# maxgillett/tinysplat

Measured on AMD Instinct MI355X. Metric: Gaussians*pixels/s fwd+bwd, higher is better.
Workload: dtype f32; 1 GPU; 1000000 random Gaussians, SH degree 3, 1920x1080, fwd+bwd (RGB), BASELINE configs[2]; max_per_tile=614, parallelism=single GPU, tile_lists=16x16 (gsplat's) (auto), gaussian_order=as generated (i.i.d.)

## Files before the change

### tinysplat_amd/csrc/raster.hip

```cpp
#include <hip/hip_runtime.h>

#include <type_traits>

#include "../../include/tinysplat_hip.h"
#include "host_util.h"
#include "raster_survivors.h"
#include "splat_math.h"

namespace {
#include "sort_network.h"

#ifndef TS_FWD_MIN_WAVES_RGB
#define TS_FWD_MIN_WAVES_RGB 5
#endif
#ifndef TS_FWD_MIN_WAVES_RGBD
#define TS_FWD_MIN_WAVES_RGBD 5
#endif
#ifndef TS_BWD_MIN_WAVES_16
#define TS_BWD_MIN_WAVES_16 5
#endif

#ifndef TS_ABLATE
#define TS_ABLATE 0
#endif

#ifndef TS_STATS
#define TS_STATS 0
#endif
#if TS_STATS
__device__ unsigned long long ts_stats[12];
#define TS_STAT(i, v)                                                                       \
    do {                                                                                    \
        if ((threadIdx.x & 63) == 0) atomicAdd(&ts_stats[i], (unsigned long long)(v));      \
    } while (0)
#else
#define TS_STAT(i, v) ((void)0)
#endif

#ifndef TS_TIMELINE
#define TS_TIMELINE 0
#endif
#if TS_TIMELINE
constexpr int kTimelineMax = 1 << 17;
constexpr int kTimelineRow = 12;
__device__ unsigned long long ts_timeline[2][kTimelineMax][kTimelineRow];
struct WaveClock {
    unsigned long long t0, c0;
    unsigned long long seg[4] = {0ull, 0ull, 0ull, 0ull};
    unsigned int work[3] = {0u, 0u, 0u};
    int which, unit, n;
    __device__ WaveClock(int which_, int unit_, int n_) : which(which_), unit(unit_), n(n_) {
        t0 = __builtin_amdgcn_s_memrealtime();
        c0 = __builtin_amdgcn_s_memtime();
    }
    __device__ ~WaveClock() {
        const unsigned long long t1 = __builtin_amdgcn_s_memrealtime();
        const unsigned long long c1 = __builtin_amdgcn_s_memtime();
        unsigned hw, xcc;
        asm volatile("s_getreg_b32 %0, hwreg(HW_REG_HW_ID)" : "=s"(hw));
        asm volatile("s_getreg_b32 %0, hwreg(HW_REG_XCC_ID)" : "=s"(xcc));
        if ((threadIdx.x & 63) == 0 && unit < kTimelineMax) {
            ts_timeline[which][unit][0] = t0;
            ts_timeline[which][unit][1] = t1;
            ts_timeline[which][unit][2] = (unsigned long long)hw | ((unsigned long long)xcc << 32);
            ts_timeline[which][unit][3] = (unsigned long long)n;
            for (int i = 0; i < 4; ++i) ts_timeline[which][unit][4 + i] = seg[i];
            ts_timeline[which][unit][8] = c1 - c0;
            for (int i = 0; i < 3; ++i) ts_timeline[which][unit][9 + i] = work[i];
        }
    }
};
#define TS_WAVE_CLOCK(which, unit, n) WaveClock ts_wave_clock_(which, unit, n)
#define TS_SEG_PARAM , unsigned long long (&ts_seg_)[4], unsigned int (&ts_work_)[3]
#define TS_SEG_ARG , ts_wave_clock_.seg, ts_wave_clock_.work
#define TS_WORK(i, v) ts_work_[i] += (unsigned int)(v)
#define TS_SEG_T0(var)                                               \
    __builtin_amdgcn_sched_barrier(0);                               \
    const unsigned long long var = __builtin_amdgcn_s_memtime();     \
    __builtin_amdgcn_sched_barrier(0)
#define TS_SEG_ADD(segs, i, var)                                     \
    __builtin_amdgcn_sched_barrier(0);                               \
    segs[i] += __builtin_amdgcn_s_memtime() - var;                   \
    __builtin_amdgcn_sched_barrier(0)
#else
#define TS_WAVE_CLOCK(which, unit, n) ((void)0)
#define TS_SEG_PARAM
#define TS_SEG_ARG
#define TS_WORK(i, v) ((void)0)
#define TS_SEG_T0(var) ((void)0)
#define TS_SEG_ADD(segs, i, var) ((void)0)
#endif

#ifndef TS_LDS_PAD
#define TS_LDS_PAD 0
#endif
#if TS_LDS_PAD
#define TS_LDS_PAD_DECL() __shared__ int lds_pad_[TS_LDS_PAD / 4]; if (threadIdx.x == 9999) lds_pad_[blockIdx.x & 7] = 1; asm volatile("" : : "v"(&lds_pad_[0]) : "memory")
#else
#define TS_LDS_PAD_DECL() ((void)0)
#endif

typedef __attribute__((address_space(3))) void* lds_ptr_t;
typedef const __attribute__((address_space(1))) void* gbl_ptr_t;
__device__ __forceinline__ void dma_record(const float4* __restrict__ splats, int g, float4* raw) {
    const float4* p = splats + 3 * (size_t)g;
    __builtin_amdgcn_global_load_lds((gbl_ptr_t)p, (lds_ptr_t)raw, 16, 0, 0);
    __builtin_amdgcn_global_load_lds((gbl_ptr_t)(p + 1), (lds_ptr_t)(raw + 64), 16, 0, 0);
    __builtin_amdgcn_global_load_lds((gbl_ptr_t)(p + 2), (lds_ptr_t)(raw + 128), 16, 0, 0);
}
#define TS_DMA_WAIT() asm volatile("s_waitcnt vmcnt(0)" ::: "memory")
#define TS_LDS_WAIT() asm volatile("s_waitcnt lgkmcnt(0)" ::: "memory")

#ifndef TS_REDUCE_AHEAD
#define TS_REDUCE_AHEAD 4
#endif

constexpr int kWaves = 4;
constexpr int kThreads = 64 * kWaves;
constexpr int kRowF4 = TS_PARTIAL_ROW_FLOATS / 4;
static_assert(TS_PARTIAL_ROW_FLOATS % 4 == 0 && TS_PARTIAL_ROW_FLOATS >= 12, "row = whole float4s, >= 10 values");
using ts::kLog2e;
using ts::kLog2_255;

#define TS_WAVE_SYNC()                                            \
    do {                                                          \
        __builtin_amdgcn_fence(__ATOMIC_RELEASE, "wavefront");    \
        __builtin_amdgcn_wave_barrier();                          \
        __builtin_amdgcn_fence(__ATOMIC_ACQUIRE, "wavefront");    \
    } while (0)

#define TS_LDS_BARRIER() asm volatile("s_waitcnt lgkmcnt(0)\n\ts_barrier" ::: "memory")

__device__ __forceinline__ int wave_max_int(int v) {
#pragma unroll
    for (int d = 32; d >= 1; d >>= 1) v = max(v, __shfl_xor(v, d, 64));
    return v;
}

__device__ __forceinline__ float sigma_l2(float hA, float B, float hC, float neg_lo, float dx, float dy) {
    float s = __builtin_fmaf(hC * dy, dy, neg_lo);
    s = __builtin_fmaf(hA * dx, dx, s);
    return __builtin_fmaf(B * dx, dy, s);
}

__device__ __forceinline__ int xcd_tile_group(int num_groups) {
    const int per_xcd = (num_groups + 7) >> 3;
    return (int)(blockIdx.x & 7) * per_xcd + (int)(blockIdx.x >> 3);
}

struct Staged {
    int mask;
    float gx, gy, hA, B, hC, lo;
};

struct BlockRect { float x0, x1, y0, y1; };
__device__ __forceinline__ bool mask_rect(unsigned long long m, int& xmin, int& xmax, int& ymin,
                                          int& ymax) {
    if (m == 0ull) return false;
    ymin = __builtin_ctzll(m) >> 3;
    ymax = (63 - __builtin_clzll(m)) >> 3;
    unsigned int c = (unsigned int)(m | (m >> 32));
    c |= c >> 16;
    c |= c >> 8;
    c &= 0xffu;
    xmin = __builtin_ctz(c);
    xmax = 31 - __builtin_clz(c);
    return true;
}

constexpr int NBC = 2, NB = NBC * NBC;
__device__ __forceinline__ Staged stage_fields(const float4 q0, const float4 q1) {
    Staged s;
    s.gx = q0.x; s.gy = q0.y;
    const float A = q0.w, Bc = q1.x, Cc = q1.y, op = q0.z;
    s.hA = 0.5f * kLog2e * A;
    s.B = kLog2e * Bc;
    s.hC = 0.5f * kLog2e * Cc;
    s.lo = __log2f(op);
    s.mask = 0;
    return s;
}
__device__ __forceinline__ Staged stage_splat(bool have, const float4 q0, const float4 q1,
                                              const float4* __restrict__ rects, int blocks) {
    Staged s = stage_fields(q0, q1);
    const float op = q0.z;
    const bool general = !(s.hA > 0.0f && s.hC > 0.0f && 4.0f * s.hA * s.hC > s.B * s.B && op <= 0.99f);
    if (have && op > 0.0f) {
        const float tau = s.lo + kLog2_255;
        if (tau >= -0.02f) {
            if (s.hA > 0.0f && s.hC > 0.0f) {
                const float inv2A = 0.5f / s.hA, inv2C = 0.5f / s.hC;
#pragma unroll 1
                for (int k = 0; k < NB; ++k) {
                    if (!(blocks & (1 << k))) continue;
                    const float4 r = rects[k];
                    if (ts::rect_may_contribute(s.hA, s.B, s.hC, inv2A, inv2C, tau, s.gx, s.gy, r.x, r.y, r.z,
                                                r.w))
                        s.mask |= (1 << k);
                }
            } else {
                s.mask = blocks;
            }
            if (s.mask != 0 && general) s.mask |= (1 << NB);
        }
    }
    return s;
}

__device__ __forceinline__ int update_rects(const bool (&sel)[NB], float X0, float Y0, float4* rects,
                                            int lane) {
    int blocks = 0;
#pragma unroll
    for (int k = 0; k < NB; ++k) {
        const unsigned long long m = __ballot(sel[k]);
        int xmin, xmax, ymin, ymax;
        if (mask_rect(m, xmin, xmax, ymin, ymax)) {
            blocks |= (1 << k);
            const float bx = X0 + (float)(8 * (k % NBC)), by = Y0 + (float)(8 * (k / NBC));
            if (lane == 0)
                rects[k] = make_float4(bx + (float)xmin, bx + (float)xmax, by + (float)ymin,
                                       by + (float)ymax);
        }
    }
    return blocks;
}

template <bool WL>
__device__ __forceinline__ int bbox_blocks(int wm, int tx) {
    const int minx = wm >> 16, w = wm & 0xffff;
    return (!WL || (tx >= minx && tx < minx + w)) ? ~0 : 0;
}

using mask64 = unsigned long long;
#define TS_BALLOT(c) __builtin_amdgcn_ballot_w64(c)
#define TS_LANE(m) __builtin_amdgcn_inverse_ballot_w64(m)

#define TS_CAM_SEGS(cam) (((cam).hints >> 8) & 15)
#ifndef TS_SEG_MIN_LIST
#define TS_SEG_MIN_LIST 65
#endif
constexpr int kSegMinList = TS_SEG_MIN_LIST;
constexpr int kSegMax = 8;
__device__ __forceinline__ int seg_bound(int list_len, int S, int s) {
    if (S <= 1 || list_len < kSegMinList) return 0x7fffff00;
    const int C = (list_len + 63) >> 6;
    int b = 0;
    for (int k = 1; k <= s; ++k) {
        const int f = (C * k * k + S * S - 1) / (S * S);
        b = max(f, b + 1);
    }
    return b << 6;
}
__host__ __device__ __forceinline__ size_t seg_plane_stride(const ts_camera& cam) {
    const int rows = min(16 * cam.tile_rows, cam.img_height - 16 * cam.tile_row0);
    return (size_t)cam.img_width * (size_t)max(rows, 0);
}

#define TS_CAM_WHOLE16(cam) (((cam).hints >> 12) & 15)
struct CutTiles {
    int band, whole;
    __host__ __device__ int cut() const { return band - whole; }
    __host__ __device__ int block_of(int tile) const {
        const int b = tile / band, j = tile - b * band;
        return j < whole ? -1 : b * (band - whole) + (j - whole);
    }
    __host__ __device__ int items(int S) const { return whole + (band - whole) * S; }
};
__host__ __device__ __forceinline__ CutTiles cut_tiles(int num_tiles, int hints) {
    CutTiles m;
    const int whole16 = (hints >> 12) & 15;
    m.band = 4 * ((num_tiles + 31) / 32);
    m.whole = whole16 > 0 ? ((m.band * whole16) / 16) & ~3 : 0;
    return m;
}
__host__ __device__ __forceinline__ size_t ckpt_offset(size_t plane) { return (plane + 63) & ~(size_t)63; }
template <int CH>
__host__ __device__ __forceinline__ size_t ckpt_record(int block, int S, int r) {
    return ((size_t)block * (size_t)S + (size_t)(r - 1)) * (size_t)((1 + CH) * 256);
}
template <int CH>
__device__ __forceinline__ void ckpt_store(float* rec, int k, int lane, float T, const float (&D)[CH]) {
    reinterpret_cast<float4*>(rec)[64 * k + lane] = make_float4(T, D[0], D[1], D[2]);
    if (CH == 4) rec[1024 + 64 * k + lane] = D[CH - 1];
}

template <int CH, int N>
struct LocRegs {
    static constexpr bool on = N > 0;
    float v[N > 0 ? N : 1][CH];
    __device__ __forceinline__ void zero() {
#pragma unroll
        for (int k = 0; k < (N > 0 ? N : 1); ++k)
#pragma unroll
            for (int c = 0; c < CH; ++c) v[k][c] = 0.0f;
    }
    __device__ __forceinline__ void add(int k, const float (&col)[CH], float vis) {
#pragma unroll
        for (int c = 0; c < CH; ++c) v[N == 1 ? 0 : k][c] = __builtin_fmaf(col[c], vis, v[N == 1 ? 0 : k][c]);
    }
    __device__ __forceinline__ void get(int k, float (&D)[CH]) const {
#pragma unroll
        for (int c = 0; c < CH; ++c) D[c] = v[N == 1 ? 0 : k][c];
    }
};
__device__ __forceinline__ float fwd_alpha(float sgl) {
    float a, ae;
    asm("v_exp_f32_e64 %0, -%2\n\t"
        "s_nop 0\n\t"
        "v_cmp_le_f32_e32 vcc, %3, %0\n\t"
        "v_cndmask_b32_e32 %1, 0, %0, vcc"
        : "=&v"(a), "=v"(ae)
        : "v"(sgl), "s"(ts::kAlphaMin)
        : "vcc");
    return ae;
}
__device__ __forceinline__ float fwd_alpha_update(float sgl, float& T, int& fidx, int idx, float& a0, float& a1, float& a2,
                                                  float c0, float c1, float c2) {
    float a, ae, nT, d, vis;
    asm("v_exp_f32_e64 %0, -%10\n\t"
        "s_nop 0\n\t"
        "v_cmp_le_f32_e32 vcc, %15, %0\n\t"
        "v_cndmask_b32_e32 %1, 0, %0, vcc\n\t"
        "v_fma_f32 %2, -%1, %5, %5\n\t"
        "v_sub_f32_e32 %3, %5, %2\n\t"
        "v_cmp_nge_f32_e32 vcc, %16, %2\n\t"
        "v_cndmask_b32_e32 %4, 0, %3, vcc\n\t"
        "v_fmac_f32_e32 %6, %11, %4\n\t"
        "v_fmac_f32_e32 %7, %12, %4\n\t"
        "v_cndmask_b32_e64 %5, -|%5|, %2, vcc\n\t"
        "v_fmac_f32_e32 %8, %13, %4\n\t"
        "v_cmp_lt_f32_e32 vcc, 0, %4\n\t"
        "v_cndmask_b32_e32 %9, %9, %14, vcc"
        : "=&v"(a), "=&v"(ae), "=&v"(nT), "=&v"(d), "=&v"(vis), "+v"(T), "+v"(a0), "+v"(a1), "+v"(a2), "+v"(fidx)
        : "v"(sgl), "v"(c0), "v"(c1), "v"(c2), "v"(idx), "s"(ts::kAlphaMin), "s"(ts::kTEps)
        : "vcc");
    return vis;
}
__device__ __forceinline__ float fwd_update(float ae, float& T, int& fidx, int idx, float& a0, float& a1, float& a2,
                                            float c0, float c1, float c2) {
    float nT, d, vis;
    asm("v_fma_f32 %0, -%8, %3, %3\n\t"
        "v_sub_f32_e32 %1, %3, %0\n\t"
        "v_cmp_nge_f32_e32 vcc, %13, %0\n\t"
        "v_cndmask_b32_e32 %2, 0, %1, vcc\n\t"
        "v_fmac_f32_e32 %4, %9, %2\n\t"
        "v_fmac_f32_e32 %5, %10, %2\n\t"
        "v_cndmask_b32_e64 %3, -|%3|, %0, vcc\n\t"
        "v_fmac_f32_e32 %6, %11, %2\n\t"
        "v_cmp_lt_f32_e32 vcc, 0, %2\n\t"
        "v_cndmask_b32_e32 %7, %7, %12, vcc"
        : "=&v"(nT), "=&v"(d), "=&v"(vis), "+v"(T), "+v"(a0), "+v"(a1), "+v"(a2), "+v"(fidx)
        : "v"(ae), "v"(c0), "v"(c1), "v"(c2), "v"(idx), "s"(ts::kTEps)
        : "vcc");
    return vis;
}

template <int CH, bool GENERAL, class Loc>
__device__ __forceinline__ void fwd_chunk(const float4* __restrict__ lds, int cnt, const float (&fpx)[NBC],
                                          const float (&fpy)[2], float (&T)[NB], int (&fidx)[NB],
                                          float (&acc)[NB][CH], Loc& loc TS_SEG_PARAM) {
#pragma clang fp contract(off)
    constexpr bool LOC = Loc::on;
    TS_WORK(0, cnt);
    for (int j = 0; j < (TS_ABLATE == 3 ? 0 : cnt); ++j) {
        TS_SEG_T0(tseg_a);
        const float4 r0 = lds[3 * j], r1 = lds[3 * j + 1], r2 = lds[3 * j + 2];
        const int bm = __builtin_amdgcn_readfirstlane(__float_as_int(r2.w));
        const int idx = __float_as_int(r2.z);
        const float neg_lo = -r1.y;
        float col[CH];
        col[0] = r1.z; col[1] = r1.w; col[2] = r2.x;
        if (CH == 4) col[CH - 1] = r2.y;
#if TS_TIMELINE
        asm volatile("s_waitcnt lgkmcnt(0)" ::: "memory");
#endif
        TS_SEG_ADD(ts_seg_, 1, tseg_a);
        TS_SEG_T0(tseg_b);
        TS_WORK(1, __popc(bm & ((1 << NB) - 1)));
#pragma unroll
        for (int k = 0; k < NB; ++k) {
            if (!(bm & (1 << k))) continue;
            if (TS_ABLATE == 5) { asm volatile("" ::: "memory"); continue; }
            TS_STAT(1, 1);
            const float sgl = sigma_l2(r0.z, r0.w, r1.x, neg_lo, r0.x - fpx[k % NBC], r0.y - fpy[k / NBC]);
            if (TS_ABLATE == 8) {
                float dup = sigma_l2(r0.z, r0.w, r1.x, neg_lo, r0.y - fpx[k % NBC], r0.x - fpy[k / NBC]);
                dup = __builtin_amdgcn_exp2f(-dup);
                asm volatile("" ::"v"(dup));
            }
            float vis;
            if (!GENERAL) {
                vis = fwd_alpha_update(sgl, T[k], fidx[k], idx, acc[k][0], acc[k][1], acc[k][2], col[0], col[1], col[2]);
            } else {
                float ae = fwd_alpha(sgl);
                ae = fminf(ts::kAlphaMax, ae);
                ae = sgl >= neg_lo ? ae : 0.0f;
                vis = fwd_update(ae, T[k], fidx[k], idx, acc[k][0], acc[k][1], acc[k][2], col[0], col[1], col[2]);
            }
            if (CH == 4) acc[k][CH - 1] = __builtin_fmaf(col[CH - 1], vis, acc[k][CH - 1]);
            if (LOC) loc.add(k, col, vis);
        }
        TS_SEG_ADD(ts_seg_, 2, tseg_b);
    }
}

#define TS_CAM_COOP16(cam) (((cam).hints >> 16) & 15)
static_assert(kWaves == 4, "a cooperative workgroup is one wave per 8x8 block of a 16x16 tile");
#ifndef TS_COOP_AHEAD
#define TS_COOP_AHEAD 4
#endif
constexpr int kCoopAhead = TS_COOP_AHEAD;
constexpr int kHintCoopAll = 1 << 21;
struct FwdPlan {
    int per_xcd;
    int coop, coop_lo;
    bool descending;
    __host__ __device__ int grid() const { return 8 * (per_xcd + (kWaves - 1) * coop); }
// ... 791 lines not shown
                }
                if ((6 + CH) & 1) acc[5 + CH] = 0.0f;
            }
        }
        TS_SEG_ADD(ts_seg_, 3, tseg_c);
    }
    if (kRowsLds) {
        TS_WAVE_SYNC();
        if (lane < cnt) {
            float4 p2 = lds[RS * lane + 2];
            if (rec_idx(p2) == kRowMark) {
                const long long slot = (long long)rec_slot(p2);
                const float4 p0 = lds[RS * lane], p1 = lds[RS * lane + 1];
                if (CH == 3) p2.y = 0.0f;
                p2.z = 0.0f; p2.w = 0.0f;
                float4* dst = reinterpret_cast<float4*>(partials) + slot * kRowF4;
                dst[0] = p0; dst[1] = p1; dst[2] = p2;
                row_flags[slot] = (unsigned char)((unsigned long long)num_isects >> 56);
            }
        }
        TS_WAVE_SYNC();
    }
}

constexpr int kBwdWaves = 1;
template <int CH, bool SPLIT, bool WL, bool SURV = false>
__global__ __launch_bounds__(64 * kBwdWaves, TS_BWD_MIN_WAVES_16) void raster_bwd_kernel(
    const ts_camera cam, const int num_tiles, const long long num_isects,
    const int* __restrict__ tile_bins, const int* __restrict__ ids_sorted,
    const float4* __restrict__ splats, const float* __restrict__ background,
    const float* __restrict__ final_Ts, const int* __restrict__ final_index,
    const float* __restrict__ v_out_img, const float* __restrict__ v_out_depth, const int planes,
    const float* __restrict__ v_out_alpha, const unsigned char* __restrict__ clamp_mask,
    float* __restrict__ partials, unsigned char* __restrict__ row_flags,
    const int* __restrict__ sv_id, const int* __restrict__ sv_meta, const int* __restrict__ sv_cnt) {
    static_assert(!SURV || (!SPLIT && !WL), "survivor lists: one wave per 16x16 tile");
    TS_LDS_PAD_DECL();
    __shared__ float4 lds_all[kBwdWaves][64 * 4];
    __shared__ float4 rect_all[kBwdWaves][NB];
    __shared__ float4 raw_all[kBwdWaves][3 * 64];
    const int wave = threadIdx.x >> 6, lane = threadIdx.x & 63;
    constexpr bool kSegs = !SPLIT && !WL;
    const int S_cam = kSegs ? max(1, min(TS_CAM_SEGS(cam), kSegMax)) : 1;
    int S_seg = S_cam, tile, seg = 0, only = -1, ck_block = -1;
    if (kSegs && S_cam > 1) {
        const CutTiles m = cut_tiles(num_tiles, cam.hints);
        const int j = (int)(blockIdx.x >> 3) * kBwdWaves + wave;
        if (j >= m.items(S_cam)) return;
        int local = j;
        S_seg = 1;
        if (j >= m.whole) {
            S_seg = S_cam;
            local = m.whole + (j - m.whole) / S_cam;
            seg = (j - m.whole) % S_cam;
        }
        tile = (int)(blockIdx.x & 7) * m.band + local;
        if (tile >= num_tiles) return;
        if (S_seg > 1) seg = (int)(((unsigned)seg + (((unsigned)tile * 2654435761u) >> 20)) % (unsigned)S_seg);
        ck_block = m.block_of(tile);
    } else {
        const int units = SPLIT ? NB * num_tiles : num_tiles;
        const int unit = xcd_tile_group((units + kBwdWaves - 1) / kBwdWaves) * kBwdWaves + wave;
        if (unit >= units) return;
        tile = SPLIT ? unit / NB : unit;
        only = SPLIT ? unit % NB : -1;
    }
    float4* rects = rect_all[wave];
    const int tbx = cam.tile_bounds_x;
    const int tx = tile % tbx, ty = tile / tbx + cam.tile_row0;
    const int list = WL ? (ty - cam.tile_row0) * ((tbx + 1) >> 1) + (tx >> 1) : tile;
    const int2 range = reinterpret_cast<const int2*>(tile_bins)[list];
    if (range.y <= range.x) return;
    int sb = range.x, se = range.y;
    bool front = false;
    const float4 zero4 = make_float4(0.f, 0.f, 0.f, 0.f);
    int id_next = 0;
    if (kSegs && S_seg > 1) {
        const int len = range.y - range.x;
        if (len < kSegMinList) {
            if (seg != 0) return;
        } else {
            sb = range.x + (seg > 0 ? seg_bound(len, S_seg, seg) : 0);
            if (sb >= range.y) return;
            se = seg + 1 < S_seg ? min(range.x + seg_bound(len, S_seg, seg + 1), range.y) : range.y;
            front = se < range.y;
        }
    }
    TS_WAVE_CLOCK(1, (int)blockIdx.x * kBwdWaves + wave, se - sb);
    float4* lds = lds_all[wave];
    const int px0 = tx * 16 + (lane & 7), py0 = ty * 16 + (lane >> 3);
    float fpx[NBC];
#pragma unroll
    for (int c = 0; c < NBC; ++c) fpx[c] = (float)(px0 + 8 * c) + ts::kPixOff;
    const float fpy[2] = {(float)py0 + ts::kPixOff, (float)(py0 + 8) + ts::kPixOff};
    const float X0 = (float)(tx * 16) + ts::kPixOff, Y0 = (float)(ty * 16) + ts::kPixOff;
    const int W = cam.img_width, H = cam.img_height;
    const int row_off = cam.tile_row0 * 16;

    float bg[CH];
#pragma unroll
    for (int c = 0; c < CH; ++c) bg[c] = background[c];

    float T[NB], R[NB], vo[NB][CH];
    int fidx[NB], bmax[NB];
    int fmax = -1;
#pragma unroll
    for (int k = 0; k < NB; ++k) {
        const int px = px0 + 8 * (k % NBC), py = py0 + 8 * (k / NBC);
        const bool inside = (px < W) && (py < H) && (!SPLIT || k == only);
        fidx[k] = -1;
        T[k] = 1.0f;
        R[k] = 0.0f;
#pragma unroll
        for (int c = 0; c < CH; ++c) vo[k][c] = 0.0f;
        if (inside) {
            const size_t pix = (size_t)(py - row_off) * W + px;
            fidx[k] = final_index[pix];
            T[k] = final_Ts[pix];
            float dotbg = 0.0f;
            float cb[CH];
#pragma unroll
            for (int c = 0; c < CH; ++c) cb[c] = 0.0f;
            float T_start = T[k];
            if (kSegs && front) {
                const float* ckp = final_Ts + ckpt_offset(seg_plane_stride(cam)) + ckpt_record<CH>(ck_block, S_cam, 1);
                T_start = ckp[(size_t)seg * ((1 + CH) * 256) + 4 * (64 * k + lane)];
                float4 d[kSegMax - 1];
                float d3[kSegMax - 1];
#pragma unroll
                for (int r = 2; r <= kSegMax; ++r) {
                    d[r - 2] = zero4;
                    d3[r - 2] = 0.0f;
                    if (r > S_seg || r < seg + 2) continue;
                    const float* rec = ckp + (size_t)(r - 1) * ((1 + CH) * 256);
                    d[r - 2] = reinterpret_cast<const float4*>(rec)[64 * k + lane];
                    if (CH == 4) d3[r - 2] = rec[1024 + 64 * k + lane];
                }
#pragma unroll
                for (int r = kSegMax; r >= 2; --r) {
                    cb[0] += d[r - 2].y; cb[1] += d[r - 2].z; cb[2] += d[r - 2].w;
                    if (CH == 4) cb[CH - 1] += d3[r - 2];
                }
            }
            const int pass = clamp_mask ? clamp_mask[pix] : 7;
#pragma unroll
            for (int c = 0; c < CH; ++c) {
                float g;
                if (CH == 4 && planes)
                    g = c < 3 ? (v_out_img ? v_out_img[pix * 3 + c] : 0.0f) : (v_out_depth ? v_out_depth[pix] : 0.0f);
                else
                    g = v_out_img[pix * CH + c];
                vo[k][c] = (c >= 3 || (pass & (1 << c))) ? g : 0.0f;
                dotbg += bg[c] * vo[k][c];
            }
            const float va = v_out_alpha ? v_out_alpha[pix] : 0.0f;
            R[k] = T[k] * (va - dotbg);
            if (kSegs && front) {
                float behind = cb[0] * vo[k][0];
#pragma unroll
                for (int c = 1; c < CH; ++c) behind = __builtin_fmaf(cb[c], vo[k][c], behind);
                R[k] -= behind;
                T[k] = T_start;
            }
        }
        bmax[k] = wave_max_int(fidx[k]);
        fmax = max(fmax, bmax[k]);
    }
    const int last = min(se - 1, fmax);
    if (last < sb) return;

    float acc[6 + CH];
#pragma unroll
    for (int c = 0; c < 6 + CH; ++c) acc[c] = 0.0f;

    float4* raw = raw_all[wave];
    if constexpr (SURV) {
        const int* cnt_t = sv_cnt + 8 * (size_t)tile;
        const int len = range.y - range.x;
        int pb = 0, pe = cnt_t[0];
        if (kSegs && S_seg > 1 && len >= kSegMinList) {
            if (seg > 0) pb = cnt_t[seg];
            if (seg + 1 < S_seg) pe = cnt_t[seg + 1];
        }
        pe = min(pe, len);
        pb = max(pb, 0);
        __shared__ int meta_all[kBwdWaves][64];
        int* meta_l = meta_all[wave];
        const int* sid = sv_id + range.x;
        const int* smeta = sv_meta + range.x;
        auto dma_meta = [&](int p) {
            __builtin_amdgcn_global_load_lds((gbl_ptr_t)(smeta + p), (lds_ptr_t)meta_l, 4, 0, 0);
        };
        if (pe - 1 - lane >= pb) {
            dma_record(splats, sid[pe - 1 - lane], raw);
            dma_meta(pe - 1 - lane);
        }
        if (pe - 65 - lane >= pb) id_next = sid[pe - 65 - lane];
        for (int hi = pe - 1; hi >= pb; hi -= 64) {
            TS_SEG_T0(tseg_p);
            const int p = hi - lane;
            const bool have = p >= pb;
            TS_DMA_WAIT();
            const float4 q0 = have ? raw[lane] : zero4, q1 = have ? raw[64 + lane] : zero4,
                         q2 = have ? raw[128 + lane] : zero4;
            const int meta = have ? meta_l[lane] : 0;
            TS_LDS_WAIT();
            if (p - 64 >= pb) {
                dma_record(splats, id_next, raw);
                dma_meta(p - 64);
            }
            if (p - 128 >= pb) id_next = sid[p - 128];
            const int i = range.x + (meta >> 8);
            int mask = meta & ((2 << NB) - 1);
#pragma unroll
            for (int k = 0; k < NB; ++k)
                if (i > bmax[k]) mask &= ~(1 << k);
            const bool keep = have && (mask & ((1 << NB) - 1)) != 0;
            const unsigned long long kmask = __ballot(keep);
            const int cnt = __popcll(kmask);
            if (keep) {
                const int pos = __popcll(kmask & ((1ull << lane) - 1ull));
                const Staged s = stage_fields(q0, q1);
                const int wm = __float_as_int(q2.w);
                const int slot = __float_as_int(q2.z) + ty * (wm & 0xffff) + tx;
                constexpr int RS = CH == 3 ? 3 : 4;
                lds[RS * pos] = make_float4(s.gx, s.gy, s.hA, s.B);
                lds[RS * pos + 1] = make_float4(s.hC, s.lo, q1.z, q1.w);
                lds[RS * pos + 2] = bwd_record_tail(q2.x, CH == 3 ? __int_as_float(mask) : q2.y, i, slot);
                if (CH == 4) lds[RS * pos + 3] = make_float4(__int_as_float(mask), 0.f, 0.f, 0.f);
            }
            TS_WAVE_SYNC();
            TS_STAT(2, cnt);
            TS_STAT(7, min(64, hi - pb + 1));
            TS_SEG_ADD(ts_wave_clock_.seg, 0, tseg_p);
            const bool general = __ballot(keep && (mask & (1 << NB))) != 0ull;
            if (general)
                bwd_chunk<CH, true>(lds, cnt, fpx, fpy, T, R, vo, fidx, acc, num_isects, partials,
                                         row_flags, lane TS_SEG_ARG);
            else
                bwd_chunk<CH, false>(lds, cnt, fpx, fpy, T, R, vo, fidx, acc, num_isects, partials,
                                          row_flags, lane TS_SEG_ARG);
            TS_WAVE_SYNC();
        }
        return;
    }
    if (last - lane >= sb) {
        const int g = ids_sorted[last - lane];
        dma_record(splats, g, raw);
    }
    if (last - 64 - lane >= sb) id_next = ids_sorted[last - 64 - lane];

    for (int hi = last; hi >= sb; hi -= 64) {
        TS_SEG_T0(tseg_p);
        const int i = hi - lane;
        const bool have = i >= sb;
        TS_DMA_WAIT();
        const float4 q0 = have ? raw[lane] : zero4, q1 = have ? raw[64 + lane] : zero4,
                     q2 = have ? raw[128 + lane] : zero4;
        TS_LDS_WAIT();
        if (i - 64 >= sb) dma_record(splats, id_next, raw);
        if (i - 128 >= sb) id_next = ids_sorted[i - 128];
        int blocks;
        {
            bool sel[NB];
#pragma unroll
            for (int k = 0; k < NB; ++k) sel[k] = fidx[k] >= hi - 63;
            blocks = update_rects(sel, X0, Y0, rects, lane);
            TS_WAVE_SYNC();
        }
        Staged s = stage_splat(have, q0, q1, rects, blocks);
        s.mask &= bbox_blocks<WL>(__float_as_int(q2.w), tx);
#pragma unroll
        for (int k = 0; k < NB; ++k)
            if (i > bmax[k]) s.mask &= ~(1 << k);
        const bool keep = (s.mask & ((1 << NB) - 1)) != 0;
        const unsigned long long mask = __ballot(keep);
        const int cnt = __popcll(mask);
        if (keep) {
            const int pos = __popcll(mask & ((1ull << lane) - 1ull));
            const int wm = __float_as_int(q2.w);
            int slot = __float_as_int(q2.z) + ty * (wm & 0xffff) + tx;
            if (SPLIT) slot = 4 * slot + only;
            constexpr int RS = CH == 3 ? 3 : 4;
            lds[RS * pos] = make_float4(s.gx, s.gy, s.hA, s.B);
            lds[RS * pos + 1] = make_float4(s.hC, s.lo, q1.z, q1.w);
            lds[RS * pos + 2] = bwd_record_tail(q2.x, CH == 3 ? __int_as_float(s.mask) : q2.y, i, slot);
            if (CH == 4) lds[RS * pos + 3] = make_float4(__int_as_float(s.mask), 0.f, 0.f, 0.f);
        }
        TS_WAVE_SYNC();
        TS_STAT(2, cnt);
        TS_STAT(7, min(64, hi - sb + 1));
        TS_SEG_ADD(ts_wave_clock_.seg, 0, tseg_p);
        const bool general = __ballot(keep && (s.mask & (1 << NB))) != 0ull;
        if (general)
            bwd_chunk<CH, true>(lds, cnt, fpx, fpy, T, R, vo, fidx, acc, num_isects, partials,
                                     row_flags, lane TS_SEG_ARG);
        else
            bwd_chunk<CH, false>(lds, cnt, fpx, fpy, T, R, vo, fidx, acc, num_isects, partials,
                                      row_flags, lane TS_SEG_ARG);
        TS_WAVE_SYNC();
    }
}

template <int CH>
__global__ __launch_bounds__(256) void reduce_partials_kernel(
    int n, int flags, const int* __restrict__ num_tiles_hit, const int* __restrict__ cum_tiles_hit,
    const float4* __restrict__ partials, const unsigned char* __restrict__ row_flags,
    const float4* __restrict__ splats, float* __restrict__ v_xy, float* __restrict__ v_conic,
    float* __restrict__ v_colors, float* __restrict__ v_opacity, float* __restrict__ v_depth,
    const unsigned char* __restrict__ color_mask, float4* __restrict__ grad_rows) {
    const int i = (int)((long long)blockIdx.x * 256 + threadIdx.x);
    if (i >= n) return;
    const int cnt = num_tiles_hit[i];
    const long long end = cum_tiles_hit[i];
    const unsigned int gen = ((unsigned int)flags >> 8) & 0xffu ? ((unsigned int)flags >> 8) & 0xffu : 1u;
    double s[10];
#pragma unroll
    for (int c = 0; c < 10; ++c) s[c] = 0.0;
    auto add_row = [&](const float4& p0, const float4& p1, const float4& p2) {
        s[0] += (double)p0.x; s[1] += (double)p0.y; s[2] += (double)p0.z; s[3] += (double)p0.w;
        s[4] += (double)p1.x; s[5] += (double)p1.y; s[6] += (double)p1.z; s[7] += (double)p1.w;
        s[8] += (double)p2.x; s[9] += (double)p2.y;
    };
    if (flags & TS_RASTER_SPLIT_BLOCKS) {
        const unsigned int* flags4 = reinterpret_cast<const unsigned int*>(row_flags);
        for (long long sl = end - cnt; sl < end; ++sl) {
            const unsigned int fw = flags4[sl];
            unsigned int f = 0u;
#pragma unroll
            for (int k = 0; k < 4; ++k) f |= (((fw >> (8 * k)) & 0xffu) == gen) ? (0xffu << (8 * k)) : 0u;
            if (f == 0u) continue;
            float4 p0[4], p1[4], p2[4];
#pragma unroll
            for (int k = 0; k < 4; ++k) {
                if (f & (0xffu << (8 * k))) {
                    p0[k] = partials[kRowF4 * (4 * sl + k)]; p1[k] = partials[kRowF4 * (4 * sl + k) + 1];
                    p2[k] = partials[kRowF4 * (4 * sl + k) + 2];
                }
            }
#pragma unroll
            for (int k = 0; k < 4; ++k) {
                if (f & (0xffu << (8 * k))) add_row(p0[k], p1[k], p2[k]);
            }
        }
    } else {
        constexpr int kAhead = TS_REDUCE_AHEAD;
        for (long long s0 = end - cnt; s0 < end; s0 += kAhead) {
            bool f[kAhead];
            float4 p0[kAhead], p1[kAhead], p2[kAhead];
#pragma unroll
            for (int u = 0; u < kAhead; ++u) f[u] = (s0 + u < end) && row_flags[s0 + u] == gen;
#pragma unroll
            for (int u = 0; u < kAhead; ++u) {
                if (f[u]) {
                    p0[u] = partials[kRowF4 * (s0 + u)]; p1[u] = partials[kRowF4 * (s0 + u) + 1];
                    p2[u] = partials[kRowF4 * (s0 + u) + 2];
                }
            }
#pragma unroll
            for (int u = 0; u < kAhead; ++u) {
                if (f[u]) add_row(p0[u], p1[u], p2[u]);
            }
        }
    }
    float4 a0 = make_float4((float)s[0], (float)s[1], (float)s[2], (float)s[3]);
    float4 a1 = make_float4((float)s[4], (float)s[5], (float)s[6], (float)s[7]);
    float4 a2 = make_float4((float)s[8], (float)s[9], 0.f, 0.f);
    float vx = 0.f, vy = 0.f, vop = 0.f;
    if (cnt > 0) {
        const float4 q0 = splats[3 * (size_t)i], q1 = splats[3 * (size_t)i + 1];
        const float A = q0.w, B = q1.x, C = q1.y, op = q0.z;
        vx = A * a0.y + B * a0.z;
        vy = B * a0.y + C * a0.z;
        vop = op > 0.0f ? -a0.x / op : 0.0f;
        if (flags & TS_RASTER_LOGIT_OPACITY) vop *= op * (1.0f - op);
        if (color_mask) {
            const int m = color_mask[i];
            if (!(m & 1)) a1.z = 0.0f;
            if (!(m & 2)) a1.w = 0.0f;
            if (!(m & 4)) a2.x = 0.0f;
        }
    }
    if (grad_rows) {
        grad_rows[3 * (size_t)i] = make_float4(vx, vy, 0.5f * a0.w, a1.x);
        grad_rows[3 * (size_t)i + 1] = make_float4(0.5f * a1.y, a1.z, a1.w, a2.x);
        grad_rows[3 * (size_t)i + 2] = make_float4(CH == 4 ? a2.y : 0.0f, vop, 0.0f, 0.0f);
        return;
    }
    reinterpret_cast<float2*>(v_xy)[i] = make_float2(vx, vy);
    v_opacity[i] = vop;
    v_conic[3 * i] = 0.5f * a0.w; v_conic[3 * i + 1] = a1.x; v_conic[3 * i + 2] = 0.5f * a1.y;
    if (CH == 4 && v_depth == nullptr) {
        reinterpret_cast<float4*>(v_colors)[i] = make_float4(a1.z, a1.w, a2.x, a2.y);
    } else if (CH == 4) {
        v_colors[3 * i] = a1.z; v_colors[3 * i + 1] = a1.w; v_colors[3 * i + 2] = a2.x;
        v_depth[i] = a2.y;
    } else {
        v_colors[3 * i] = a1.z; v_colors[3 * i + 1] = a1.w; v_colors[3 * i + 2] = a2.x;
    }
}

}

extern "C" {

#if TS_TIMELINE
int ts_debug_timeline(unsigned long long* out_host, int which, int count) {
    if (which < 0 || which > 1 || count < 0 || count > kTimelineMax) return TS_E_BADARG;
    return (int)hipMemcpyFromSymbol(out_host, HIP_SYMBOL(ts_timeline), (size_t)count * kTimelineRow * 8,
                                    (size_t)which * kTimelineMax * kTimelineRow * 8);
}
#endif

#if TS_STATS
int ts_debug_stats(unsigned long long* out_host, int reset) {
    hipError_t e = hipMemcpyFromSymbol(out_host, HIP_SYMBOL(ts_stats), sizeof(ts_stats));
    if (e == hipSuccess && reset) {
        unsigned long long z[12] = {0};
        e = hipMemcpyToSymbol(HIP_SYMBOL(ts_stats), z, sizeof(z));
    }
    return (int)e;
}
#endif

int64_t ts_final_floats(const ts_camera* cam, int32_t channels) {
    if (!cam || (channels != 3 && channels != 4)) return TS_E_BADARG;
    const size_t plane = seg_plane_stride(*cam);
    const int S = min(TS_CAM_SEGS(*cam), kSegMax);
    if (S <= 1 || cam->wide_tiles) return (int64_t)plane;
    const CutTiles m = cut_tiles(ts_num_tiles(cam), cam->hints);
    return (int64_t)(ckpt_offset(plane) + (size_t)8 * (size_t)m.cut() * (size_t)(S * (1 + channels) * 256));
}

int32_t ts_cut_tiles(const ts_camera* cam, int32_t* band, int32_t* whole) {
    if (!cam) return TS_E_BADARG;
    const CutTiles m = cut_tiles(ts_num_tiles(cam), cam->hints);
    if (band) *band = m.band;
    if (whole) *whole = m.whole;
    return 8 * m.cut();
}

int ts_raster_fwd(int32_t channels, int32_t flags, const ts_camera* cam, const int32_t* tile_bins,
                  const int32_t* gaussian_ids_sorted, const float* splats, const float* background,
                  float* out_img, float* final_Ts, int32_t* final_index, uint8_t* clamp_mask,
                  void* stream) {
    return ts_raster_fwd_planes(channels, flags, cam, tile_bins, gaussian_ids_sorted, splats, background, out_img,
                                nullptr, final_Ts, final_index, clamp_mask, stream);
}

int ts_raster_fwd_planes(int32_t channels, int32_t flags, const ts_camera* cam, const int32_t* tile_bins,
                         const int32_t* gaussian_ids_sorted, const float* splats, const float* background,
                         float* out_img, float* out_depth, float* final_Ts, int32_t* final_index,
                         uint8_t* clamp_mask, void* stream) {
    if (!cam || (channels != 3 && channels != 4) || (out_depth && channels != 4)) return TS_E_BADARG;
    const bool narrow = cam->wide_tiles != 0;
    if (narrow && !(flags & TS_RASTER_NARROW_WAVES)) return TS_E_BADARG;
    const int nt = narrow ? cam->tile_rows * cam->tile_bounds_x : ts_num_tiles(cam);
    if (nt <= 0) return 0;
    if (!tile_bins || !background || !out_img || (!final_Ts != !final_index)) return TS_E_BADARG;
    bool split = (flags & TS_RASTER_SPLIT_BLOCKS) != 0;
    ts_camera kcam = *cam;
    kcam.hints &= ~kHintCoopAll;
    if (split && !narrow && (cam->hints & TS_HINT_COOP_SPLIT)) {
        split = false;
        kcam.hints |= kHintCoopAll;
    }
    const int units = split ? 4 * nt : nt;
    int grid = 8 * (((units + kWaves - 1) / kWaves + 7) / 8);
    hipStream_t s = (hipStream_t)stream;
    const float4* sp = reinterpret_cast<const float4*>(splats);
    const int clamp = (flags & TS_RASTER_CLAMP_RGB) ? 1 : 0;
    const bool segs = !narrow && final_Ts && TS_CAM_SEGS(*cam) > 1;
    if (!split && !narrow) grid = fwd_plan(nt, kcam.hints, segs, true).grid();
#define TS_LAUNCH_FWD(C, S, L, G)                                                                  \
    hipLaunchKernelGGL((raster_fwd_kernel<C, S, L, false, G>), dim3(grid), dim3(kThreads), 0, s, kcam, nt, \
                       tile_bins, gaussian_ids_sorted, (const int*)nullptr, (const float*)nullptr,   \
                       (int*)nullptr, sp, background, out_img, out_depth, final_Ts,                  \
                       final_index, clamp, clamp ? clamp_mask : nullptr, (int*)nullptr, (int*)nullptr, (int*)nullptr)
#define TS_LAUNCH_FWD_X(C, S)                                                                      \
    do {                                                                                           \
        if (narrow) TS_LAUNCH_FWD(C, S, true, false);                                              \
        else if (segs) TS_LAUNCH_FWD(C, S, false, true);                                           \
        else TS_LAUNCH_FWD(C, S, false, false);                                                    \
    } while (0)
    if (channels == 3) { if (split) TS_LAUNCH_FWD_X(3, true); else TS_LAUNCH_FWD_X(3, false); }
    else { if (split) TS_LAUNCH_FWD_X(4, true); else TS_LAUNCH_FWD_X(4, false); }
#undef TS_LAUNCH_FWD_X
#undef TS_LAUNCH_FWD
    return launch_status();
}

int ts_raster_fwd_sort(int32_t channels, int32_t flags, const ts_camera* cam, const int32_t* tile_bins,
                       const int32_t* bucket_ids, const float* depths, int32_t* gaussian_ids_sorted,
                       const float* splats, const float* background, float* out_img, float* out_depth,
                       float* final_Ts, int32_t* final_index, uint8_t* clamp_mask, void* stream) {
    return ts_surv::raster_fwd_sort(channels, flags, cam, tile_bins, bucket_ids, depths, gaussian_ids_sorted, splats,
                                    background, out_img, out_depth, final_Ts, final_index, clamp_mask, nullptr, stream);
}

int ts_raster_bwd(int32_t channels, int32_t flags, int64_t num_intersects, const ts_camera* cam,
                  const int32_t* tile_bins, const int32_t* gaussian_ids_sorted, const float* splats,
                  const float* background, const float* final_Ts, const int32_t* final_index,
                  const float* v_out_img, const float* v_out_alpha, const uint8_t* clamp_mask,
                  float* partials, uint8_t* row_flags, void* stream) {
    return ts_raster_bwd_planes(channels, flags, num_intersects, cam, tile_bins, gaussian_ids_sorted, splats, background,
                                final_Ts, final_index, v_out_img, nullptr, 0, v_out_alpha, clamp_mask, partials,
                                row_flags, stream);
}

int ts_raster_bwd_planes(int32_t channels, int32_t flags, int64_t num_intersects, const ts_camera* cam,
                         const int32_t* tile_bins, const int32_t* gaussian_ids_sorted, const float* splats,
                         const float* background, const float* final_Ts, const int32_t* final_index,
                         const float* v_out_img, const float* v_out_depth, int32_t planes,
                         const float* v_out_alpha, const uint8_t* clamp_mask,
                         float* partials, uint8_t* row_flags, void* stream) {
    return ts_surv::raster_bwd(channels, flags, num_intersects, cam, tile_bins, gaussian_ids_sorted, splats, background,
                               final_Ts, final_index, v_out_img, v_out_depth, planes, v_out_alpha, clamp_mask, partials,
                               row_flags, nullptr, nullptr, stream);
}

}

namespace ts_surv {

int raster_fwd_sort(int32_t channels, int32_t flags, const ts_camera* cam, const int32_t* tile_bins,
                    const int32_t* bucket_ids, const float* depths, int32_t* gaussian_ids_sorted,
                    const float* splats, const float* background, float* out_img, float* out_depth,
                    float* final_Ts, int32_t* final_index, uint8_t* clamp_mask, int32_t* survivors, void* stream) {
    if (!cam || (channels != 3 && channels != 4) || (out_depth && channels != 4)) return TS_E_BADARG;
    if (cam->wide_tiles != 0 || (flags & TS_RASTER_NARROW_WAVES)) return TS_E_BADARG;
    const int nt = ts_num_tiles(cam);
    if (nt <= 0) return 0;
    if (!tile_bins || !background || !out_img || (!final_Ts != !final_index) || !bucket_ids || !depths ||
        !gaussian_ids_sorted)
        return TS_E_BADARG;
    bool split = (flags & TS_RASTER_SPLIT_BLOCKS) != 0;
    if (survivors && (split || !final_Ts)) return TS_E_BADARG;
    ts_camera kcam = *cam;
    kcam.hints &= ~kHintCoopAll;
    if (split && (cam->hints & TS_HINT_COOP_SPLIT)) {
        split = false;
        kcam.hints |= kHintCoopAll;
    }
    const int units = split ? 4 * nt : nt;
    int grid = 8 * (((units + kWaves - 1) / kWaves + 7) / 8);
    hipStream_t s = (hipStream_t)stream;
    const float4* sp = reinterpret_cast<const float4*>(splats);
    const int clamp = (flags & TS_RASTER_CLAMP_RGB) ? 1 : 0;
    const bool segs = final_Ts && TS_CAM_SEGS(*cam) > 1;
    if (!split) grid = fwd_plan(nt, kcam.hints, segs, true).grid();
    int* sv_id = survivors ? const_cast<int*>(bucket_ids) : nullptr;
    int* sv_cnt = survivors;
    int* sv_meta = survivors ? survivors + survivor_counts(nt) : nullptr;
#define TS_LAUNCH_FWD_SORT(C, S, G, V)                                                                            \
    hipLaunchKernelGGL((raster_fwd_kernel<C, S, false, true, G, V>), dim3(grid), dim3(kThreads), 0, s, kcam, nt,    \
                       tile_bins, (const int*)nullptr, bucket_ids, depths, gaussian_ids_sorted, sp, background, \
                       out_img, out_depth, final_Ts, final_index, clamp, clamp ? clamp_mask : nullptr, sv_id, sv_meta, \
                       sv_cnt)
    if (channels == 3) {
        if (split && segs) TS_LAUNCH_FWD_SORT(3, true, true, false);
        else if (split) TS_LAUNCH_FWD_SORT(3, true, false, false);
        else if (segs && survivors) TS_LAUNCH_FWD_SORT(3, false, true, true);
        else if (segs) TS_LAUNCH_FWD_SORT(3, false, true, false);
        else if (survivors) TS_LAUNCH_FWD_SORT(3, false, false, true);
        else TS_LAUNCH_FWD_SORT(3, false, false, false);
    } else {
        if (split && segs) TS_LAUNCH_FWD_SORT(4, true, true, false);
        else if (split) TS_LAUNCH_FWD_SORT(4, true, false, false);
        else if (segs && survivors) TS_LAUNCH_FWD_SORT(4, false, true, true);
        else if (segs) TS_LAUNCH_FWD_SORT(4, false, true, false);
        else if (survivors) TS_LAUNCH_FWD_SORT(4, false, false, true);
        else TS_LAUNCH_FWD_SORT(4, false, false, false);
    }
#undef TS_LAUNCH_FWD_SORT
    return launch_status();
}

int raster_bwd(int32_t channels, int32_t flags, int64_t num_intersects, const ts_camera* cam,
               const int32_t* tile_bins, const int32_t* gaussian_ids_sorted, const float* splats,
               const float* background, const float* final_Ts, const int32_t* final_index,
               const float* v_out_img, const float* v_out_depth, int32_t planes,
               const float* v_out_alpha, const uint8_t* clamp_mask,
               float* partials, uint8_t* row_flags, const int32_t* bucket_ids, const int32_t* survivors,
               void* stream) {
    if (!cam || (channels != 3 && channels != 4) || num_intersects < 0) return TS_E_BADARG;
    if (survivors && (!bucket_ids || (flags & (TS_RASTER_SPLIT_BLOCKS | TS_RASTER_NARROW_WAVES)) || cam->wide_tiles))
        return TS_E_BADARG;
    if (planes ? channels != 4 : v_out_depth != nullptr) return TS_E_BADARG;
    const bool narrow = cam->wide_tiles != 0;
    if (narrow && !(flags & TS_RASTER_NARROW_WAVES)) return TS_E_BADARG;
    const int nt = narrow ? cam->tile_rows * cam->tile_bounds_x : ts_num_tiles(cam);
    if (nt <= 0 || num_intersects == 0) return 0;
    if (!tile_bins || !gaussian_ids_sorted || !splats || !background || !final_Ts || !final_index ||
        (!planes && !v_out_img) || !partials || !row_flags)
        return TS_E_BADARG;
    hipStream_t s = (hipStream_t)stream;
    const bool split = (flags & TS_RASTER_SPLIT_BLOCKS) != 0;
    const int gen = (flags >> 8) & 0xff;
    if (gen == 0) {
        hipError_t e = hipMemsetAsync(row_flags, 0, (size_t)num_intersects * (split ? 4 : 1), s);
        if (e != hipSuccess) return (int)e;
    }
    const long long isects_tagged = (long long)(((unsigned long long)(gen ? gen : 1) << 56) |
                                                ((unsigned long long)num_intersects & 0x00ffffffffffffffull));
    if (TS_CAM_SEGS(*cam) < 0 || TS_CAM_SEGS(*cam) > kSegMax) return TS_E_BADARG;
    const int segs = (!split && !narrow && TS_CAM_SEGS(*cam) > 1) ? TS_CAM_SEGS(*cam) : 1;
    int grid;
    if (segs > 1) {
        const CutTiles m = cut_tiles(nt, cam->hints);
        grid = 8 * ((m.items(segs) + kBwdWaves - 1) / kBwdWaves);
    } else {
        const int units = split ? 4 * nt : nt;
        grid = 8 * (((units + kBwdWaves - 1) / kBwdWaves + 7) / 8);
    }
    const float4* sp = reinterpret_cast<const float4*>(splats);
    const int* sv_cnt = survivors;
    const int* sv_meta = survivors ? survivors + survivor_counts(nt) : nullptr;
#define TS_LAUNCH_BWD(C, S, L, V)                                                                  \
    hipLaunchKernelGGL((raster_bwd_kernel<C, S, L, V>), dim3(grid), dim3(64 * kBwdWaves), 0, s, *cam, nt, \
                       isects_tagged, tile_bins, gaussian_ids_sorted, sp, background,              \
                       final_Ts, final_index, v_out_img, v_out_depth, planes ? 1 : 0, v_out_alpha,  \
                       clamp_mask, partials, row_flags, bucket_ids, sv_meta, sv_cnt)
#define TS_LAUNCH_BWD_X(C, S)                                                                      \
    do {                                                                                           \
        if (narrow) TS_LAUNCH_BWD(C, S, true, false);                                              \
        else if (survivors) TS_LAUNCH_BWD(C, false, false, true);               \
        else TS_LAUNCH_BWD(C, S, false, false);                                                    \
    } while (0)
    if (channels == 3) { if (split) TS_LAUNCH_BWD_X(3, true); else TS_LAUNCH_BWD_X(3, false); }
    else { if (split) TS_LAUNCH_BWD_X(4, true); else TS_LAUNCH_BWD_X(4, false); }
#undef TS_LAUNCH_BWD_X
#undef TS_LAUNCH_BWD
    return launch_status();
}

}

extern "C" {

int ts_reduce_partials(int32_t n, int32_t channels, int32_t flags, const int32_t* num_tiles_hit,
                       const int32_t* cum_tiles_hit, const float* partials,
                       const uint8_t* row_flags, const float* splats, float* v_xy, float* v_conic,
                       float* v_colors, float* v_opacity, float* v_depth, const uint8_t* color_mask,
                       void* stream) {
    if (n < 0 || (channels != 3 && channels != 4)) return TS_E_BADARG;
    if (n == 0) return 0;
    if (!num_tiles_hit || !cum_tiles_hit || !row_flags || !splats || !v_xy || !v_conic || !v_colors || !v_opacity)
        return TS_E_BADARG;
    hipStream_t s = (hipStream_t)stream;
    const float4* pr = reinterpret_cast<const float4*>(partials);
    const float4* sp = reinterpret_cast<const float4*>(splats);
    const int grid = (int)(((long long)n + 255) / 256);
    if (channels == 3)
        hipLaunchKernelGGL(reduce_partials_kernel<3>, dim3(grid), dim3(256), 0, s, n, (int)flags, num_tiles_hit,
                           cum_tiles_hit, pr, row_flags, sp, v_xy, v_conic, v_colors, v_opacity, v_depth, color_mask,
                           (float4*)nullptr);
    else
        hipLaunchKernelGGL(reduce_partials_kernel<4>, dim3(grid), dim3(256), 0, s, n, (int)flags, num_tiles_hit,
                           cum_tiles_hit, pr, row_flags, sp, v_xy, v_conic, v_colors, v_opacity, v_depth, color_mask,
                           (float4*)nullptr);
    return launch_status();
}

int ts_reduce_partials_rows(int32_t n, int32_t channels, int32_t flags, const int32_t* num_tiles_hit,
                            const int32_t* cum_tiles_hit, const float* partials, const uint8_t* row_flags,
                            const float* splats, float* grad_rows, void* stream) {
    if (n < 0 || (channels != 3 && channels != 4)) return TS_E_BADARG;
    if (n == 0) return 0;
    if (!num_tiles_hit || !cum_tiles_hit || !row_flags || !splats || !grad_rows) return TS_E_BADARG;
    hipStream_t s = (hipStream_t)stream;
    const float4* pr = reinterpret_cast<const float4*>(partials);
    const float4* sp = reinterpret_cast<const float4*>(splats);
    float4* gr = reinterpret_cast<float4*>(grad_rows);
    const int grid = (int)(((long long)n + 255) / 256);
    if (channels == 3)
        hipLaunchKernelGGL(reduce_partials_kernel<3>, dim3(grid), dim3(256), 0, s, n, (int)flags, num_tiles_hit,
                           cum_tiles_hit, pr, row_flags, sp, (float*)nullptr, (float*)nullptr, (float*)nullptr,
                           (float*)nullptr, (float*)nullptr, (const unsigned char*)nullptr, gr);
    else
        hipLaunchKernelGGL(reduce_partials_kernel<4>, dim3(grid), dim3(256), 0, s, n, (int)flags, num_tiles_hit,
                           cum_tiles_hit, pr, row_flags, sp, (float*)nullptr, (float*)nullptr, (float*)nullptr,
                           (float*)nullptr, (float*)nullptr, (const unsigned char*)nullptr, gr);
    return launch_status();
}

}
```

Before: 2093000 billion Gaussians*pixels/s.

## Scan reduce-partials row flags as bitmasks and gather only live rows

The non-split reduce path now loads 32 row flags at once with vector loads, turns them into a bitmask with SWAR byte compares, and gathers partial rows only for set bits, four at a time. The next flag window is requested while the current gathers are in flight. The split/non-split choice becomes a template parameter, and the splat loads are hoisted to the kernel start to overlap latency. This removes per-row byte flag loads and wasted loop iterations over dead rows, at the cost of more complex control flow and over-reading flag memory near buffer edges.

```diff
diff --git a/tinysplat_amd/csrc/raster.hip b/tinysplat_amd/csrc/raster.hip
--- a/tinysplat_amd/csrc/raster.hip
+++ b/tinysplat_amd/csrc/raster.hip
@@ -111,8 +111,11 @@
 #define TS_DMA_WAIT() asm volatile("s_waitcnt vmcnt(0)" ::: "memory")
 #define TS_LDS_WAIT() asm volatile("s_waitcnt lgkmcnt(0)" ::: "memory")
 
-#ifndef TS_REDUCE_AHEAD
-#define TS_REDUCE_AHEAD 4
+#ifndef TS_REDUCE_ROWS
+#define TS_REDUCE_ROWS 4
+#endif
+#ifndef TS_REDUCE_BLOCK
+#define TS_REDUCE_BLOCK 256
 #endif
 
 constexpr int kWaves = 4;
@@ -1510,17 +1513,50 @@
     }
 }
 
-template <int CH>
-__global__ __launch_bounds__(256) void reduce_partials_kernel(
+
+struct FlagWindow {
+    uint4 c0, c1, c2;
+    int sh, len;
+
+    __device__ __forceinline__ void request(const unsigned char* __restrict__ row_flags, int s0, int end) {
+        sh = (int)((unsigned long long)(row_flags + s0) & 15ull);
+        len = min(32, end - s0);
+        const unsigned char* p = row_flags + ((long long)s0 - sh);
+        c0 = *reinterpret_cast<const uint4*>(p);
+        c1 = *reinterpret_cast<const uint4*>(p + (sh + len > 16 ? 16 : 0));
+        c2 = *reinterpret_cast<const uint4*>(p + (sh + len > 32 ? 32 : 0));
+    }
+    static __device__ __forceinline__ unsigned int piece_bits(const uint4& c, unsigned int gen4) {
+        auto nibble = [gen4](unsigned int w) {
+            w ^= gen4;
+            const unsigned int nz = ((w & 0x7f7f7f7fu) + 0x7f7f7f7fu) | w;
+            return (((~nz & 0x80808080u) >> 7) * 0x01020408u) >> 24;
+        };
+        return nibble(c.x) | (nibble(c.y) << 4) | (nibble(c.z) << 8) | (nibble(c.w) << 12);
+    }
+    __device__ __forceinline__ unsigned int bits(unsigned int gen4) const {
+        const unsigned long long b = (unsigned long long)piece_bits(c0, gen4) |
+                                     ((unsigned long long)piece_bits(c1, gen4) << 16) |
+                                     ((unsigned long long)piece_bits(c2, gen4) << 32);
+        return (unsigned int)(b >> sh) & (0xffffffffu >> (32 - len));
+    }
+};
+
+constexpr int kReduceBlock = TS_REDUCE_BLOCK;
+
+template <int CH, bool SPLIT>
+__global__ __launch_bounds__(kReduceBlock) void reduce_partials_kernel(
     int n, int flags, const int* __restrict__ num_tiles_hit, const int* __restrict__ cum_tiles_hit,
     const float4* __restrict__ partials, const unsigned char* __restrict__ row_flags,
     const float4* __restrict__ splats, float* __restrict__ v_xy, float* __restrict__ v_conic,
     float* __restrict__ v_colors, float* __restrict__ v_opacity, float* __restrict__ v_depth,
     const unsigned char* __restrict__ color_mask, float4* __restrict__ grad_rows) {
-    const int i = (int)((long long)blockIdx.x * 256 + threadIdx.x);
+    const int i = (int)((long long)blockIdx.x * kReduceBlock + threadIdx.x);
     if (i >= n) return;
-    const int cnt = num_tiles_hit[i];
-    const long long end = cum_tiles_hit[i];
+    int cnt = num_tiles_hit[i], end32 = cum_tiles_hit[i];
+    const float4 q0 = splats[3 * (size_t)i], q1 = splats[3 * (size_t)i + 1];
+    asm volatile("" : "+v"(cnt), "+v"(end32));
+    const long long end = end32;
     const unsigned int gen = ((unsigned int)flags >> 8) & 0xffu ? ((unsigned int)flags >> 8) & 0xffu : 1u;
     double s[10];
 #pragma unroll
@@ -1530,7 +1566,7 @@
         s[4] += (double)p1.x; s[5] += (double)p1.y; s[6] += (double)p1.z; s[7] += (double)p1.w;
         s[8] += (double)p2.x; s[9] += (double)p2.y;
     };
-    if (flags & TS_RASTER_SPLIT_BLOCKS) {
+    if (SPLIT) {
         const unsigned int* flags4 = reinterpret_cast<const unsigned int*>(row_flags);
         for (long long sl = end - cnt; sl < end; ++sl) {
             const unsigned int fw = flags4[sl];
@@ -1552,23 +1588,39 @@
             }
         }
     } else {
-        constexpr int kAhead = TS_REDUCE_AHEAD;
-        for (long long s0 = end - cnt; s0 < end; s0 += kAhead) {
-            bool f[kAhead];
-            float4 p0[kAhead], p1[kAhead], p2[kAhead];
-#pragma unroll
-            for (int u = 0; u < kAhead; ++u) f[u] = (s0 + u < end) && row_flags[s0 + u] == gen;
-#pragma unroll
-            for (int u = 0; u < kAhead; ++u) {
-                if (f[u]) {
-                    p0[u] = partials[kRowF4 * (s0 + u)]; p1[u] = partials[kRowF4 * (s0 + u) + 1];
-                    p2[u] = partials[kRowF4 * (s0 + u) + 2];
+        constexpr int kRows = TS_REDUCE_ROWS;
+        const unsigned int gen4 = gen * 0x01010101u;
+        const int last = (int)end;
+        int s0 = last - cnt;
+        FlagWindow win;
+        unsigned int m = 0u;
+        bool more = cnt > 0;
+        if (more) { win.request(row_flags, s0, last); m = win.bits(gen4); }
+        while (more) {
+            more = s0 + 32 < last;
+            do {
+                bool f[kRows];
+                long long row[kRows];
+                float4 p0[kRows], p1[kRows], p2[kRows];
+#pragma unroll
+                for (int r = 0; r < kRows; ++r) {
+                    f[r] = m != 0u;
+                    row[r] = (long long)kRowF4 * (s0 + (__ffs(m) - 1));
+                    m &= m - 1u;
                 }
-            }
-#pragma unroll
-            for (int u = 0; u < kAhead; ++u) {
-                if (f[u]) add_row(p0[u], p1[u], p2[u]);
-            }
+#pragma unroll
+                for (int r = 0; r < kRows; ++r) asm volatile("" : "+v"(row[r]));
+#pragma unroll
+                for (int r = 0; r < kRows; ++r) {
+                    if (f[r]) { p0[r] = partials[row[r]]; p1[r] = partials[row[r] + 1]; p2[r] = partials[row[r] + 2]; }
+                }
+                if (m == 0u && more) win.request(row_flags, s0 + 32, last);
+#pragma unroll
+                for (int r = 0; r < kRows; ++r) {
+                    if (f[r]) add_row(p0[r], p1[r], p2[r]);
+                }
+            } while (m);
+            if (more) { s0 += 32; m = win.bits(gen4); }
         }
     }
     float4 a0 = make_float4((float)s[0], (float)s[1], (float)s[2], (float)s[3]);
@@ -1576,7 +1628,6 @@
     float4 a2 = make_float4((float)s[8], (float)s[9], 0.f, 0.f);
     float vx = 0.f, vy = 0.f, vop = 0.f;
     if (cnt > 0) {
-        const float4 q0 = splats[3 * (size_t)i], q1 = splats[3 * (size_t)i + 1];
         const float A = q0.w, B = q1.x, C = q1.y, op = q0.z;
         vx = A * a0.y + B * a0.z;
         vy = B * a0.y + C * a0.z;
@@ -1844,6 +1895,26 @@
 
 }
 
+namespace {
+
+void launch_reduce_partials(int32_t n, int32_t channels, int32_t flags, const int32_t* num_tiles_hit,
+                            const int32_t* cum_tiles_hit, const float* partials, const uint8_t* row_flags,
+                            const float* splats, float* v_xy, float* v_conic, float* v_colors, float* v_opacity,
+                            float* v_depth, const uint8_t* color_mask, float* grad_rows, void* stream) {
+    const int grid = (int)(((long long)n + kReduceBlock - 1) / kReduceBlock);
+#define TS_LAUNCH_REDUCE(CH, SPLIT)                                                                                     \
+    hipLaunchKernelGGL((reduce_partials_kernel<CH, SPLIT>), dim3(grid), dim3(kReduceBlock), 0, (hipStream_t)stream, n,  \
+                       (int)flags, num_tiles_hit, cum_tiles_hit, reinterpret_cast<const float4*>(partials), row_flags,  \
+                       reinterpret_cast<const float4*>(splats), v_xy, v_conic, v_colors, v_opacity, v_depth, color_mask, \
+                       reinterpret_cast<float4*>(grad_rows))
+    const bool split = (flags & TS_RASTER_SPLIT_BLOCKS) != 0;
+    if (channels == 3) { if (split) TS_LAUNCH_REDUCE(3, true); else TS_LAUNCH_REDUCE(3, false); }
+    else { if (split) TS_LAUNCH_REDUCE(4, true); else TS_LAUNCH_REDUCE(4, false); }
+#undef TS_LAUNCH_REDUCE
+}
+
+}
+
 extern "C" {
 
 int ts_reduce_partials(int32_t n, int32_t channels, int32_t flags, const int32_t* num_tiles_hit,
@@ -1855,18 +1926,8 @@
     if (n == 0) return 0;
     if (!num_tiles_hit || !cum_tiles_hit || !row_flags || !splats || !v_xy || !v_conic || !v_colors || !v_opacity)
         return TS_E_BADARG;
-    hipStream_t s = (hipStream_t)stream;
-    const float4* pr = reinterpret_cast<const float4*>(partials);
-    const float4* sp = reinterpret_cast<const float4*>(splats);
-    const int grid = (int)(((long long)n + 255) / 256);
-    if (channels == 3)
-        hipLaunchKernelGGL(reduce_partials_kernel<3>, dim3(grid), dim3(256), 0, s, n, (int)flags, num_tiles_hit,
-                           cum_tiles_hit, pr, row_flags, sp, v_xy, v_conic, v_colors, v_opacity, v_depth, color_mask,
-                           (float4*)nullptr);
-    else
-        hipLaunchKernelGGL(reduce_partials_kernel<4>, dim3(grid), dim3(256), 0, s, n, (int)flags, num_tiles_hit,
-                           cum_tiles_hit, pr, row_flags, sp, v_xy, v_conic, v_colors, v_opacity, v_depth, color_mask,
-                           (float4*)nullptr);
+    launch_reduce_partials(n, channels, flags, num_tiles_hit, cum_tiles_hit, partials, row_flags, splats, v_xy, v_conic,
+                           v_colors, v_opacity, v_depth, color_mask, nullptr, stream);
     return launch_status();
 }
 
@@ -1876,19 +1937,8 @@
     if (n < 0 || (channels != 3 && channels != 4)) return TS_E_BADARG;
     if (n == 0) return 0;
     if (!num_tiles_hit || !cum_tiles_hit || !row_flags || !splats || !grad_rows) return TS_E_BADARG;
-    hipStream_t s = (hipStream_t)stream;
-    const float4* pr = reinterpret_cast<const float4*>(partials);
-    const float4* sp = reinterpret_cast<const float4*>(splats);
-    float4* gr = reinterpret_cast<float4*>(grad_rows);
-    const int grid = (int)(((long long)n + 255) / 256);
-    if (channels == 3)
-        hipLaunchKernelGGL(reduce_partials_kernel<3>, dim3(grid), dim3(256), 0, s, n, (int)flags, num_tiles_hit,
-                           cum_tiles_hit, pr, row_flags, sp, (float*)nullptr, (float*)nullptr, (float*)nullptr,
-                           (float*)nullptr, (float*)nullptr, (const unsigned char*)nullptr, gr);
-    else
-        hipLaunchKernelGGL(reduce_partials_kernel<4>, dim3(grid), dim3(256), 0, s, n, (int)flags, num_tiles_hit,
-                           cum_tiles_hit, pr, row_flags, sp, (float*)nullptr, (float*)nullptr, (float*)nullptr,
-                           (float*)nullptr, (float*)nullptr, (const unsigned char*)nullptr, gr);
+    launch_reduce_partials(n, channels, flags, num_tiles_hit, cum_tiles_hit, partials, row_flags, splats, nullptr, nullptr,
+                           nullptr, nullptr, nullptr, nullptr, grad_rows, stream);
     return launch_status();
 }
 
```

After: 2116000 billion Gaussians*pixels/s (median of 6 runs). +1.1%, better.
